# reazon-research/ReazonSpeech

Measured on AMD Instinct MI355X. Metric: RTFx (audio-sec/wall-sec), FastConformer-RNNT 619M batch=256, higher is better.
Workload: dtype bf16

## Files before the change

reazonspeech_amd/csrc/k_frontend.hip:

```cpp
#include "rs_common.h"
#include "k_fft512.h"

namespace {

constexpr int NFFT = FFT512_N;
constexpr int NBIN = FFT512_NBIN;
constexpr int FB_MAXW = 32;
constexpr int WAVES = 4;
constexpr int FRAMES_PER_WAVE = 4;
constexpr int MAX_HOP = 256;
constexpr int SPAN_MAX = (WAVES * FRAMES_PER_WAVE - 1) * MAX_HOP + NFFT;

struct FrontParams {
    const float* audio; const int32_t* lens; float* raw; int32_t* n_frames;
    const float* window;
    const float* twiddle;
    const int32_t* fb_idx;
    const float* fb_w;
    int audio_stride, pad_left, pad_right, t_max, n_mels, win_length, hop;
    float preemph, log_guard;
    int kind;
};

__device__ __forceinline__ float fetch_sample(const float* __restrict__ a, int i, int pad_left, int len) {
    const int j = i - pad_left;
    return (j >= 0 && j < len) ? a[j] : 0.0f;
}

__global__ __launch_bounds__(64 * WAVES) void logmel_kernel(FrontParams p) {
    __shared__ float2 buf[WAVES][FFT512_BUF];
    __shared__ float pw[WAVES][2][NBIN + 3];
    __shared__ float2 tw[NFFT / 2];
    __shared__ float ys[SPAN_MAX];
    __shared__ float win_s[NFFT];
    const int lane = threadIdx.x & 63, wave = threadIdx.x >> 6;
    const int b = blockIdx.y;
    const int len = p.lens[b];
    const int Lp = len + p.pad_left + p.pad_right;
    const int n_valid = p.kind == 2 ? (Lp + p.hop / 2) / p.hop
                                    : Lp / p.hop + (p.kind == 1 ? 1 : 0);
    if (blockIdx.x == 0 && threadIdx.x == 0) p.n_frames[b] = n_valid;
    const float* a = p.audio + (size_t)b * p.audio_stride;
    if ((int)blockIdx.x * WAVES * FRAMES_PER_WAVE >= min(n_valid, p.t_max)) return;
    tw[threadIdx.x] = reinterpret_cast<const float2*>(p.twiddle)[threadIdx.x];
    const int centre_off = (NFFT - p.win_length) / 2;
    const int f0 = blockIdx.x * WAVES * FRAMES_PER_WAVE;
    const int i_base = p.kind == 2 ? f0 * p.hop + p.hop / 2 - p.win_length / 2 : f0 * p.hop - NFFT / 2 + centre_off;
    const int span = (WAVES * FRAMES_PER_WAVE - 1) * p.hop + NFFT;
    for (int idx = threadIdx.x; idx < span; idx += blockDim.x) {
        int i = i_base + idx;
        float y = 0.0f;
        if (p.kind == 1 && Lp > 1) {
            i = i < 0 ? -i : i;
            i = i >= Lp ? 2 * (Lp - 1) - i : i;
            i = i < 0 ? 0 : i;
        }
        if (p.kind == 2 && Lp > 0) {
            for (int bounce = 0; bounce < 8 && (i < 0 || i >= Lp); ++bounce) i = i < 0 ? -i - 1 : 2 * Lp - 1 - i;
            i = i < 0 ? 0 : (i >= Lp ? Lp - 1 : i);
        }
        if (i >= 0 && i < Lp) {
            const float x0 = fetch_sample(a, i, p.pad_left, len);
            if (p.kind == 2) y = x0;
            else y = i >= 1 ? x0 - p.preemph * fetch_sample(a, i - 1, p.pad_left, len) : x0;
        }
        ys[idx] = y;
    }
    for (int idx = threadIdx.x; idx < NFFT; idx += blockDim.x) win_s[idx] = idx < p.win_length ? p.window[idx] : 0.0f;
    __syncthreads();
    const int frame_base = (blockIdx.x * WAVES + wave) * FRAMES_PER_WAVE;
    auto wave_sync = [&]() { fft512_wave_sync(); };
    auto sample = [&](int t, int n) -> float {
        if (t >= n_valid || t >= p.t_max) return 0.0f;
        return ys[(t - f0) * p.hop + n] * win_s[n];
    };
    auto frame_mean = [&](int t) -> float {
        if (t >= n_valid || t >= p.t_max) return 0.0f;
        float sm = 0.0f;
        for (int n = lane; n < p.win_length; n += 64) sm += ys[(t - f0) * p.hop + n];
        return wave_sum(sm) / (float)p.win_length;
    };
    auto sample_kaldi = [&](int t, int n, float mean) -> float {
        if (t >= n_valid || t >= p.t_max || n >= p.win_length) return 0.0f;
        const float* fr = ys + (t - f0) * p.hop;
        const float cur = fr[n] - mean, prev = fr[n > 0 ? n - 1 : 0] - mean;
        return (cur - p.preemph * prev) * win_s[n];
    };

    for (int fi = 0; fi < FRAMES_PER_WAVE; fi += 2) {
        const int t = frame_base + fi;
        if (t >= n_valid || t >= p.t_max) break;
        float2* z = buf[wave];
        float2 v[8];
        if (p.kind == 2) {
            const float m0 = frame_mean(t), m1 = frame_mean(t + 1);
#pragma unroll
            for (int k = 0; k < 8; ++k) v[k] = make_float2(sample_kaldi(t, lane + 64 * k, m0), sample_kaldi(t + 1, lane + 64 * k, m1));
        } else {
#pragma unroll
            for (int k = 0; k < 8; ++k) v[k] = make_float2(sample(t, lane + 64 * k), sample(t + 1, lane + 64 * k));
        }
        fft512_pair(v, z, tw, lane);
        fft512_split_power(z, pw[wave][0], pw[wave][1], lane);
        for (int idx = lane; idx < 2 * p.n_mels; idx += 64) {
            const int f = idx >= p.n_mels, m = idx - f * p.n_mels;
            if (t + f < n_valid && t + f < p.t_max) {
                const int k0 = p.fb_idx[2 * m], cnt = p.fb_idx[2 * m + 1];
                const float* w = p.fb_w + m * FB_MAXW;
                float acc = 0.0f;
                for (int j = 0; j < cnt; ++j) acc = fmaf(w[j], pw[wave][f][k0 + j], acc);
                p.raw[((size_t)b * p.t_max + t + f) * p.n_mels + m] = p.kind >= 1 ? logf(fmaxf(acc, p.log_guard)) : logf(acc + p.log_guard);
            }
        }
        wave_sync();
    }
}

__global__ __launch_bounds__(1024) void feat_normalize_kernel(const float* __restrict__ raw,
                                                              const int32_t* __restrict__ n_frames, int t_max,
                                                              int n_mels, float eps, float* __restrict__ out) {
    __shared__ float4 red[1024];
    __shared__ float4 mean_s[32], rstd_s[32];
    const int b = blockIdx.x;
    const int n = min(n_frames[b], t_max);
    const int Q = n_mels >> 2;
    const int RG = 1000 / Q;
    const int tid = threadIdx.x;
    const int q = tid % Q, rg = tid / Q;
    const bool act = rg < RG;
    const float4* r4 = reinterpret_cast<const float4*>(raw + (size_t)b * t_max * n_mels);
    auto reduce_rows = [&](float4 v) -> float4 {
        red[tid] = act ? v : make_float4(0.f, 0.f, 0.f, 0.f);
        __syncthreads();
        float4 acc = make_float4(0.f, 0.f, 0.f, 0.f);
        if (tid < Q) {
            for (int g = 0; g < RG; ++g) {
                const float4 x = red[g * Q + tid];
                acc.x += x.x; acc.y += x.y; acc.z += x.z; acc.w += x.w;
            }
        }
        return acc;
    };
    float4 s = make_float4(0.f, 0.f, 0.f, 0.f);
    if (act)
#pragma unroll 8
        for (int t = rg; t < n; t += RG) {
            const float4 x = r4[(size_t)t * Q + q];
            s.x += x.x; s.y += x.y; s.z += x.z; s.w += x.w;
        }
    s = reduce_rows(s);
    if (tid < Q) {
        const float inv = 1.0f / (float)n;
        mean_s[tid] = make_float4(s.x * inv, s.y * inv, s.z * inv, s.w * inv);
    }
    __syncthreads();
    const float4 mean = mean_s[q];
    float4 m2 = make_float4(0.f, 0.f, 0.f, 0.f);
    if (act)
#pragma unroll 8
        for (int t = rg; t < n; t += RG) {
            const float4 x = r4[(size_t)t * Q + q];
            const float a = x.x - mean.x, bb = x.y - mean.y, c = x.z - mean.z, d = x.w - mean.w;
            m2.x += a * a; m2.y += bb * bb; m2.z += c * c; m2.w += d * d;
        }
    m2 = reduce_rows(m2);
    if (tid < Q) {
        const float dn = (float)(n - 1);
        rstd_s[tid] = n > 1 ? make_float4(1.0f / (sqrtf(m2.x / dn) + eps), 1.0f / (sqrtf(m2.y / dn) + eps),
                                          1.0f / (sqrtf(m2.z / dn) + eps), 1.0f / (sqrtf(m2.w / dn) + eps))
                            : make_float4(0.f, 0.f, 0.f, 0.f);
    }
    __syncthreads();
    const float4 rstd = rstd_s[q];
    float4* o4 = reinterpret_cast<float4*>(out + (size_t)b * t_max * n_mels);
    if (act)
#pragma unroll 8
        for (int t = rg; t < t_max; t += RG) {
            float4 y = make_float4(0.f, 0.f, 0.f, 0.f);
            if (t < n) {
                const float4 x = r4[(size_t)t * Q + q];
                y = make_float4((x.x - mean.x) * rstd.x, (x.y - mean.y) * rstd.y, (x.z - mean.z) * rstd.z,
                                (x.w - mean.w) * rstd.w);
            }
            o4[(size_t)t * Q + q] = y;
        }
}

__global__ __launch_bounds__(256) void feat_mvn_kernel(const float* __restrict__ raw, const int32_t* __restrict__ n_frames, int t_max,
                                                       int n_mels, const float* __restrict__ mean, const float* __restrict__ istd,
                                                       float* __restrict__ out) {
    const int b = blockIdx.y;
    const int i = blockIdx.x * 256 + threadIdx.x;
    if (i >= t_max * n_mels) return;
    const int t = i / n_mels, m = i - t * n_mels;
    const size_t at = (size_t)b * t_max * n_mels + i;
    out[at] = t < n_frames[b] ? (raw[at] - mean[m]) * istd[m] : 0.0f;
}

}

int rs_launch_frontend(rs_ctx* ctx, const float* audio, const int32_t* lens, int B, int audio_stride,
                       int pad_left, int pad_right, int t_max, float* feats, int32_t* n_frames, float* raw,
                       hipStream_t s) {
    const rs_dims& d = ctx->d;
    if (B <= 0 || t_max <= 0) return RS_OK;
    if (d.n_fft != NFFT) return rs_fail(ctx, RS_EINVAL, "frontend: only n_fft=512 is built");
    if (d.n_mels > 128 || d.n_mels % 4 || d.win_length > NFFT || d.hop_length < 1 || d.hop_length > MAX_HOP)
        return rs_fail(ctx, RS_EINVAL, "frontend: n_mels must be a multiple of 4 up to 128, win <= 512, hop <= %d", MAX_HOP);
    FrontParams p;
    p.audio = audio; p.lens = lens; p.raw = raw; p.n_frames = n_frames;
    p.window = ctx->fe_window; p.twiddle = ctx->fe_twiddle; p.fb_idx = ctx->fe_fb_idx; p.fb_w = ctx->fe_fb_w;
    p.audio_stride = audio_stride; p.pad_left = pad_left; p.pad_right = pad_right; p.t_max = t_max;
    p.n_mels = d.n_mels; p.win_length = d.win_length; p.hop = d.hop_length;
    p.preemph = d.preemph; p.log_guard = d.log_guard;
    p.kind = d.frontend_kind;
    const int fpb = WAVES * FRAMES_PER_WAVE;
    const dim3 grid((t_max + fpb - 1) / fpb, B), block(64 * WAVES);
    if (d.frontend_kind == 2) {
        p.raw = feats;
        RS_HIP(ctx, hipMemsetAsync(feats, 0, (size_t)B * t_max * d.n_mels * 4, s));
    }
    const double bytes = (double)B * ((double)t_max * d.hop_length * 4.0 + (double)t_max * d.n_mels * 4.0 * 3.0);
    rs_prof_scope prof(ctx, RS_PROF_FRONTEND, s, (double)B * t_max * (5.0 * 512 * 9 + 3 * 257 + 2 * 600), bytes);
    hipLaunchKernelGGL(logmel_kernel, grid, block, 0, s, p);
    if (d.frontend_kind == 2) {
    } else if (d.frontend_kind == 1) {
        const rs_conformer& cf = *rs_conformer_of(ctx);
        hipLaunchKernelGGL(feat_mvn_kernel, dim3((t_max * d.n_mels + 255) / 256, B), dim3(256), 0, s, raw, n_frames, t_max, d.n_mels,
                           cf.fe_mvn_mean, cf.fe_mvn_istd, feats);
    } else
        hipLaunchKernelGGL(feat_normalize_kernel, dim3(B), dim3(1024), 0, s, raw, n_frames, t_max, d.n_mels, d.norm_eps,
                           feats);
    prof.end();
    RS_CHECK_LAUNCH(ctx, "frontend");
    return RS_OK;
}
```

reazonspeech_amd/csrc/k_subsample.hip:

```cpp
#include "rs_common.h"

namespace {

__global__ void enc_lens_kernel(const int32_t* __restrict__ n_frames, int B, int stages, int sub_kind, int32_t* __restrict__ out) {
    const int b = blockIdx.x * blockDim.x + threadIdx.x;
    if (b >= B) return;
    int n = n_frames[b];
    for (int s = 0; s < stages; ++s) {
        n = n > 0 ? (sub_kind ? (n >= 3 ? (n - 3) / 2 + 1 : 0) : (n + 2 - 3) / 2 + 1) : 0;
        out[s * B + b] = n;
    }
}

__device__ __forceinline__ void put(uint16_t* p, float v) { *p = f32_to_bf16(v); }
__device__ __forceinline__ void put(float* p, float v) { *p = v; }

template <typename OT>
__global__ __launch_bounds__(256) void sub_conv0_dw1_kernel(
    const float* __restrict__ feats, const int32_t* __restrict__ lens_stage , int B, int t_max,
    int n_mels, int T2, int F1, int F2, int C, const float* __restrict__ w0 ,
    const float* __restrict__ b0, const float* __restrict__ wd , const float* __restrict__ bd,
    OT* __restrict__ out) {
    const int b = blockIdx.y, t2 = blockIdx.x, c = threadIdx.x;
    const int L1 = lens_stage[0 * B + b], L2 = lens_stage[1 * B + b];
    OT* orow = out + (((size_t)b * T2 + t2) * F2) * C + c;
    if (t2 >= L2) {
        for (int f2 = 0; f2 < F2; ++f2) put(orow + (size_t)f2 * C, 0.0f);
        return;
    }
    float k0[9], kd[9];
#pragma unroll
    for (int j = 0; j < 9; ++j) { k0[j] = w0[j * C + c]; kd[j] = wd[j * C + c]; }
    const float bias0 = b0[c], biasd = bd[c];
    const float* fb = feats + (size_t)b * t_max * n_mels;

    const float* rowp[7];
    bool rowok[7];
#pragma unroll
    for (int r = 0; r < 7; ++r) {
        const int tm = 4 * t2 - 3 + r;
        rowok[r] = tm >= 0 && tm < t_max;
        rowp[r] = fb + (size_t)(tm < 0 ? 0 : (tm >= t_max ? t_max - 1 : tm)) * n_mels;
    }
    float kz[3][9];
    bool a_ok[3];
#pragma unroll
    for (int a = 0; a < 3; ++a) {
        const int t1 = 2 * t2 - 1 + a;
        a_ok[a] = t1 >= 0 && t1 < L1;
#pragma unroll
        for (int i = 0; i < 3; ++i)
#pragma unroll
            for (int j = 0; j < 3; ++j) kz[a][i * 3 + j] = rowok[2 * a + i] ? k0[i * 3 + j] : 0.0f;
    }
    float carry[7];
#pragma unroll
    for (int r = 0; r < 7; ++r) carry[r] = 0.0f;
    float left[3];
#pragma unroll
    for (int a = 0; a < 3; ++a) left[a] = 0.0f;
    for (int f2 = 0; f2 < F2; ++f2) {
        float m[7][5];
#pragma unroll
        for (int r = 0; r < 7; ++r) {
            const float4 q = *reinterpret_cast<const float4*>(rowp[r] + 4 * f2);
            m[r][0] = carry[r]; m[r][1] = q.x; m[r][2] = q.y; m[r][3] = q.z; m[r][4] = q.w;
            carry[r] = q.w;
        }
        float mid[3], right[3];
#pragma unroll
        for (int a = 0; a < 3; ++a) {
            float am = 0.0f, ar = 0.0f;
            if (a_ok[a]) {
                am = bias0; ar = bias0;
#pragma unroll
                for (int i = 0; i < 3; ++i)
#pragma unroll
                    for (int j = 0; j < 3; ++j) {
                        am = fmaf(kz[a][i * 3 + j], m[2 * a + i][j], am);
                        ar = fmaf(kz[a][i * 3 + j], m[2 * a + i][2 + j], ar);
                    }
                am = fmaxf(am, 0.0f); ar = fmaxf(ar, 0.0f);
            }
            mid[a] = am; right[a] = ar;
        }
        float acc = biasd;
#pragma unroll
        for (int a = 0; a < 3; ++a) {
            acc = fmaf(kd[a * 3 + 0], left[a], acc);
            acc = fmaf(kd[a * 3 + 1], mid[a], acc);
            acc = fmaf(kd[a * 3 + 2], right[a], acc);
        }
        put(orow + (size_t)f2 * C, acc);
#pragma unroll
        for (int a = 0; a < 3; ++a) left[a] = right[a];
    }
}

__global__ __launch_bounds__(256) void sub_dw_kernel(const uint16_t* __restrict__ in, const float* __restrict__ w ,
                                                     const float* __restrict__ bias, const int32_t* __restrict__ lens_out,
                                                     int Tin, int Fin, int Tout, int Fout, int C,
                                                     uint16_t* __restrict__ out) {
    const int cgs = C >> 3;
    const int cg = threadIdx.x % cgs, fl = threadIdx.x / cgs, fpb = blockDim.x / cgs;
    const int fo = blockIdx.x * fpb + fl, to = blockIdx.y, b = blockIdx.z;
    if (fo >= Fout) return;
    const int c = cg * 8;
    uint16_t* op = out + (((size_t)b * Tout + to) * Fout + fo) * C + c;
    u16x8_t o;
    if (to >= lens_out[b]) {
#pragma unroll
        for (int e = 0; e < 8; ++e) o[e] = 0;
        *reinterpret_cast<u16x8_t*>(op) = o;
        return;
    }
    float acc[8];
    {
        const float4 b0 = reinterpret_cast<const float4*>(bias + c)[0], b1 = reinterpret_cast<const float4*>(bias + c)[1];
        acc[0] = b0.x; acc[1] = b0.y; acc[2] = b0.z; acc[3] = b0.w; acc[4] = b1.x; acc[5] = b1.y; acc[6] = b1.z; acc[7] = b1.w;
    }
#pragma unroll
    for (int i = 0; i < 3; ++i) {
        const int ti = 2 * to - 1 + i;
        if (ti < 0 || ti >= Tin) continue;
#pragma unroll
        for (int j = 0; j < 3; ++j) {
            const int fi = 2 * fo - 1 + j;
            if (fi < 0 || fi >= Fin) continue;
            const u16x8_t x = *reinterpret_cast<const u16x8_t*>(in + (((size_t)b * Tin + ti) * Fin + fi) * C + c);
            const float4 w0 = reinterpret_cast<const float4*>(w + (i * 3 + j) * C + c)[0];
            const float4 w1 = reinterpret_cast<const float4*>(w + (i * 3 + j) * C + c)[1];
            acc[0] = fmaf(w0.x, bf16_to_f32(x[0]), acc[0]); acc[1] = fmaf(w0.y, bf16_to_f32(x[1]), acc[1]);
            acc[2] = fmaf(w0.z, bf16_to_f32(x[2]), acc[2]); acc[3] = fmaf(w0.w, bf16_to_f32(x[3]), acc[3]);
            acc[4] = fmaf(w1.x, bf16_to_f32(x[4]), acc[4]); acc[5] = fmaf(w1.y, bf16_to_f32(x[5]), acc[5]);
            acc[6] = fmaf(w1.z, bf16_to_f32(x[6]), acc[6]); acc[7] = fmaf(w1.w, bf16_to_f32(x[7]), acc[7]);
        }
    }
#pragma unroll
    for (int e = 0; e < 8; ++e) o[e] = f32_to_bf16(acc[e]);
    *reinterpret_cast<u16x8_t*>(op) = o;
}

__global__ __launch_bounds__(256) void sub_dw_f32_kernel(const float* __restrict__ in, const float* __restrict__ w ,
                                                         const float* __restrict__ bias, const int32_t* __restrict__ lens_out,
                                                         int Tin, int Fin, int Tout, int Fout, int C, float* __restrict__ out) {
    const int c = threadIdx.x, fo = blockIdx.x, to = blockIdx.y, b = blockIdx.z;
    float* op = out + (((size_t)b * Tout + to) * Fout + fo) * C + c;
    if (to >= lens_out[b]) { *op = 0.0f; return; }
    float acc = bias[c];
#pragma unroll
    for (int i = 0; i < 3; ++i) {
        const int ti = 2 * to - 1 + i;
        if (ti < 0 || ti >= Tin) continue;
#pragma unroll
        for (int j = 0; j < 3; ++j) {
            const int fi = 2 * fo - 1 + j;
            if (fi < 0 || fi >= Fin) continue;
            acc = fmaf(w[(i * 3 + j) * C + c], in[(((size_t)b * Tin + ti) * Fin + fi) * C + c], acc);
        }
    }
    *op = acc;
}

}

int rs_launch_enc_lens(rs_ctx* ctx, const int32_t* n_frames, int B, int32_t* lens_out, hipStream_t s) {
    hipLaunchKernelGGL(enc_lens_kernel, dim3((B + 127) / 128), dim3(128), 0, s, n_frames, B, ctx->d.sub_stages, ctx->d.sub_kind, lens_out);
    RS_CHECK_LAUNCH(ctx, "enc_lens");
    return RS_OK;
}

int rs_launch_sub_conv0_dw1(rs_ctx* ctx, const float* feats, const int32_t* lens_stage, int B, int t_max, int T2,
                            int F2, uint16_t* out, hipStream_t s) {
    const rs_dims& d = ctx->d;
    const rs_conformer& cf = *rs_conformer_of(ctx);
    const int C = d.sub_channels;
    if (C > 256 || (C % 64)) return rs_fail(ctx, RS_EINVAL, "subsampling: channels %d unsupported (<=256, %%64)", C);
    const int F1 = (d.n_mels + 2 - 3) / 2 + 1;
    if (d.n_mels % 4 || 4 * F2 > d.n_mels || 2 * F2 < F1)
        return rs_fail(ctx, RS_EINVAL, "subsampling: n_mels=%d must be a multiple of 4 with 4*F2 <= n_mels", d.n_mels);
    const size_t lds = 0;
    const double flops = (double)B * T2 * F2 * C * 2.0 * (6 * 9 + 9);
    const double bytes = (double)B * t_max * d.n_mels * 4.0 + (double)B * T2 * F2 * C * 2.0;
    rs_prof_scope prof(ctx, RS_PROF_SUBSAMPLE, s, flops, bytes);
    hipLaunchKernelGGL(sub_conv0_dw1_kernel<uint16_t>, dim3(T2, B), dim3(C), lds, s, feats, lens_stage, B, t_max, d.n_mels, T2,
                       F1, F2, C, cf.sub_conv0_w, cf.sub_conv0_b, cf.sub_dw_w[0], cf.sub_dw_b[0], out);
    prof.end();
    RS_CHECK_LAUNCH(ctx, "sub_conv0_dw1");
    return RS_OK;
}

int rs_launch_sub_dw(rs_ctx* ctx, const uint16_t* in, const float* w, const float* b, const int32_t* lens_out,
                     int stage, int B, int t_in, int f_in, int t_out, int f_out, uint16_t* out, hipStream_t s) {
    (void)stage;
    const int C = ctx->d.sub_channels;
    const int cgs = C / 8;
    const int fpb = 256 / cgs;
    const dim3 grid((f_out + fpb - 1) / fpb, t_out, B), block(cgs * fpb);
    const double bytes = (double)B * C * 2.0 * ((double)t_in * f_in + (double)t_out * f_out);
    rs_prof_scope prof(ctx, RS_PROF_SUBSAMPLE, s, (double)B * t_out * f_out * C * 18.0, bytes);
    hipLaunchKernelGGL(sub_dw_kernel, grid, block, 0, s, in, w, b, lens_out, t_in, f_in, t_out, f_out, C, out);
    prof.end();
    RS_CHECK_LAUNCH(ctx, "sub_dw");
    return RS_OK;
}

int rs_launch_sub_conv0_dw1_f32(rs_ctx* ctx, const float* feats, const int32_t* lens_stage, int B, int t_max, int T2, int F2,
                                float* out, hipStream_t s) {
    const rs_dims& d = ctx->d;
    const rs_conformer& cf = *rs_conformer_of(ctx);
    const int C = d.sub_channels;
    if (C > 256 || (C % 64)) return rs_fail(ctx, RS_EINVAL, "subsampling: channels %d unsupported (<=256, %%64)", C);
    const int F1 = (d.n_mels + 2 - 3) / 2 + 1;
    if (d.n_mels % 4 || 4 * F2 > d.n_mels || 2 * F2 < F1)
        return rs_fail(ctx, RS_EINVAL, "subsampling: n_mels=%d must be a multiple of 4 with 4*F2 <= n_mels", d.n_mels);
    rs_prof_scope prof(ctx, RS_PROF_SUBSAMPLE, s, (double)B * T2 * F2 * C * 2.0 * (6 * 9 + 9),
                       (double)B * t_max * d.n_mels * 4.0 + (double)B * T2 * F2 * C * 4.0);
    hipLaunchKernelGGL(sub_conv0_dw1_kernel<float>, dim3(T2, B), dim3(C), 0, s, feats, lens_stage, B, t_max, d.n_mels, T2, F1, F2, C,
                       cf.sub_conv0_w, cf.sub_conv0_b, cf.sub_dw_w[0], cf.sub_dw_b[0], out);
    prof.end();
    RS_CHECK_LAUNCH(ctx, "sub_conv0_dw1_f32");
    return RS_OK;
}

int rs_launch_sub_dw_f32(rs_ctx* ctx, const float* in, const float* w, const float* b, const int32_t* lens_out, int B, int t_in,
                         int f_in, int t_out, int f_out, float* out, hipStream_t s) {
    const int C = ctx->d.sub_channels;
    rs_prof_scope prof(ctx, RS_PROF_SUBSAMPLE, s, (double)B * t_out * f_out * C * 18.0,
                       (double)B * C * 4.0 * ((double)t_in * f_in + (double)t_out * f_out));
    hipLaunchKernelGGL(sub_dw_f32_kernel, dim3(f_out, t_out, B), dim3(C), 0, s, in, w, b, lens_out, t_in, f_in, t_out, f_out, C, out);
    prof.end();
    RS_CHECK_LAUNCH(ctx, "sub_dw_f32");
    return RS_OK;
}
```

reazonspeech_amd/csrc/rs_knobs.h:

```cpp
#pragma once
#include <stdlib.h>
#include <string.h>

#include <atomic>
#include <mutex>

#include "../../include/rs_asr.h"

#define RS_KNOBS(X)                                                                                                                   \
    X(GEMM_TILE, "RS_GEMM_TILE", INT, 0, "forced GEMM tile height (256 / 192 / 128 / 64); 0 = by shape")                              \
    X(GEMM_GROUP_M, "RS_GEMM_GROUP_M", INT, 0, "row panels per XCD tile group; 0 = by shape")                                         \
    X(GEMM_PAIRS, "RS_GEMM_PAIRS", INT, 2, "2 = two tiles per workgroup, LDS ring carried over; 1 = ring restarted; 0 = one tile")    \
    X(GEMM_BREG, "RS_GEMM_BREG", INT, 0, "1 = 256- / 192-row launches keep the weight operand out of LDS (global -> VGPR)")           \
    X(ATTN_PERSIST, "RS_ATTN_PERSIST", INT, 0, "1 = full attention on resident workgroups that walk the items (n >= 2: on n)")        \
    X(ATTN_STREAM, "RS_ATTN_STREAM", INT, 0, "1 = the streaming attention form (+ 16 x mask: phases left out, for timing)")           \
    X(ATTN64, "RS_ATTN64", INT, 4, "head_dim 64: key blocks per chunk; 0 = the one-workgroup-per-CU geometry")                        \
    X(ATTN64_NW, "RS_ATTN64_NW", INT, 4, "head_dim 64: waves per workgroup (the second number of $RS_ATTN64)")                        \
    X(ATTN_F32_OLD, "RS_ATTN_F32_OLD", PRESENT, 0, "float32 attention: the first form (one wave per key sum)")                        \
    X(ATTN_F32_KEYS, "RS_ATTN_F32_KEYS", PRESENT, 0, "float32 attention: the second form (keys over lanes, no MFMA)")                 \
    X(GLU_GENERIC, "RS_GLU_GENERIC", INT, 0, "GLU + depthwise conv: 1 = the any-kernel-size path, 2 = the f32-tile kernel on the gated layout") \
    X(SUB_IM2COL, "RS_SUB_IM2COL", PRESENT, 0, "ESPnet subsampling: gather the 3 x 3 patches into a matrix first (sizes the workspace too)") \
    X(FUSE_GLU, "RS_FUSE_GLU", INT, 1, "context default: 0 = GLU in the depthwise kernel, not the pw1 GEMM epilogue")                 \
    X(DEFER_OUT_NORM, "RS_DEFER_OUT_NORM", INT, 1, "context default: 0 = every output norm stores its f32 rows")                      \
    X(DECODE_SCREEN, "RS_DECODE_SCREEN", INT, 1, "context default: 0 = exact evaluation of every joint column")                       \
    X(DECODE_NARROW, "RS_DECODE_NARROW", INT, 1, "context default: 0 = the wide-tile LSTM / projection kernels")                      \
    X(DECODE_NO_XCD, "RS_DECODE_NO_XCD", PRESENT, 0, "greedy decode: joint grids not padded to a multiple of 8 column tiles")         \
    X(DECODE_NO_LOOKAHEAD, "RS_DECODE_NO_LOOKAHEAD", PRESENT, 0, "greedy decode: one frame per utterance and step at every batch size") \
    X(VERIFY_WIDE, "RS_VERIFY_WIDE", INT, 0, "screened joint: 1 = a workgroup per row for V <= 3072 too")                             \
    X(DECODE_TRACE, "RS_DECODE_TRACE", PRESENT, 0, "greedy decode: print the step count of every call to stderr")                     \
    X(BEAM_SPEC, "RS_BEAM_SPEC", INT, 3, "beam search: evaluations asked for per iteration (1 .. 8; sizes the workspace too)")         \
    X(BEAM_TRACE, "RS_BEAM_TRACE", PRESENT, 0, "beam search: phase timing of the step kernel")                                        \
    X(BEAM_RECORD_LDS, "RS_BEAM_RECORD_LDS", PRESENT, 0, "beam search: the any-vocabulary record kernel on a small vocabulary")       \
    X(AVSR_POSCONV_OLD, "RS_AVSR_POSCONV_OLD", PRESENT, 0, "AV-HuBERT positional convolution: the VALU form")                         \
    X(K2_CONV1_OLD, "RS_K2_CONV1_OLD", PRESENT, 0, "Zipformer conv1: the VALU form (the one other channel counts run)")               \
    X(K2_ATTW_SWEEPS, "RS_K2_ATTW_SWEEPS", INT, 1, "Zipformer attention weights: 3 = the three-sweep kernel")                         \
    X(K2_CONV2_FUSED, "RS_K2_CONV2_FUSED", INT, 1, "default of option k2_conv2_fused: 0 = patch matrix + GEMM launch")                \
    X(K2_CNX_FUSED, "RS_K2_CNX_FUSED", INT, 1, "default of option k2_cnx_fused: 0 = the ConvNeXt pointwise pair as two GEMM launches")

enum rs_knob_id {
#define RS_KNOB_ENUM(id, env, kind, def, what) RS_KNOB_##id,
    RS_KNOBS(RS_KNOB_ENUM)
#undef RS_KNOB_ENUM
    RS_KNOB_COUNT
};
enum rs_knob_kind { RS_KNOB_PRESENT, RS_KNOB_INT };
struct rs_knob_row { const char* env; rs_knob_kind kind; int def; };
static const rs_knob_row rs_knob_rows[RS_KNOB_COUNT] = {
#define RS_KNOB_ROW(id, env, kind, def, what) {env, RS_KNOB_##kind, def},
    RS_KNOBS(RS_KNOB_ROW)
#undef RS_KNOB_ROW
};

struct rs_knob_table {
    std::atomic<int> value[RS_KNOB_COUNT];
    std::atomic<bool> given[RS_KNOB_COUNT];
    std::once_flag once;
};
inline rs_knob_table rs_knob_state;

inline void rs_knobs_read_env() {
    std::call_once(rs_knob_state.once, [] {
        rs_knob_table& t = rs_knob_state;
        for (int i = 0; i < RS_KNOB_COUNT; ++i) { t.value[i] = rs_knob_rows[i].def; t.given[i] = false; }
        for (int i = 0; i < RS_KNOB_COUNT; ++i) {
            const char* e = i == RS_KNOB_ATTN64_NW ? nullptr : getenv(rs_knob_rows[i].env);
            if (!e) continue;
            t.given[i] = true;
            t.value[i] = rs_knob_rows[i].kind == RS_KNOB_PRESENT ? 1 : atoi(e);
            if (i == RS_KNOB_ATTN64) {
                t.given[RS_KNOB_ATTN64_NW] = true;
                if (const char* c = strchr(e, ',')) t.value[RS_KNOB_ATTN64_NW] = atoi(c + 1);
            }
        }
    });
}

inline int rs_knob(rs_knob_id id) { rs_knobs_read_env(); return rs_knob_state.value[id].load(std::memory_order_relaxed); }
inline bool rs_knob_given(rs_knob_id id) { rs_knobs_read_env(); return rs_knob_state.given[id].load(std::memory_order_relaxed); }
inline void rs_knob_set(rs_knob_id id, int v) { rs_knobs_read_env(); rs_knob_state.value[id].store(v, std::memory_order_relaxed); }

inline int rs_knob_find(const char* env_name) {
    for (int i = 0; env_name && i < RS_KNOB_COUNT; ++i)
        if (!strcmp(env_name, rs_knob_rows[i].env)) return i;
    return -1;
}
inline int rs_knob_set_named(const char* env_name, int v) {
    const int i = rs_knob_find(env_name);
    if (i < 0) return RS_EINVAL;
    rs_knob_set((rs_knob_id)i, v);
    return RS_OK;
}
inline int rs_knob_get_named(const char* env_name, int* v) {
    const int i = rs_knob_find(env_name);
    if (i < 0 || !v) return RS_EINVAL;
    *v = rs_knob((rs_knob_id)i);
    return RS_OK;
}
```

Before: 45670.

## Add lean log-mel and row-run subsampling kernels reusing conv rows across time

```diff
diff --git a/reazonspeech_amd/csrc/k_frontend.hip b/reazonspeech_amd/csrc/k_frontend.hip
--- a/reazonspeech_amd/csrc/k_frontend.hip
+++ b/reazonspeech_amd/csrc/k_frontend.hip
@@ -27,12 +27,17 @@
     return (j >= 0 && j < len) ? a[j] : 0.0f;
 }
 
+constexpr int MEL_PASSES = 4;
+template <bool LEAN>
 __global__ __launch_bounds__(64 * WAVES) void logmel_kernel(FrontParams p) {
     __shared__ float2 buf[WAVES][FFT512_BUF];
     __shared__ float pw[WAVES][2][NBIN + 3];
     __shared__ float2 tw[NFFT / 2];
-    __shared__ float ys[SPAN_MAX];
-    __shared__ float win_s[NFFT];
+    __shared__ float ys_first[LEAN ? 1 : SPAN_MAX];
+    __shared__ float win_first[LEAN ? 1 : NFFT];
+    extern __shared__ float lean_lds[];
+    float* const ys = LEAN ? lean_lds : ys_first;
+    float* const win_s = win_first;
     const int lane = threadIdx.x & 63, wave = threadIdx.x >> 6;
     const int b = blockIdx.y;
     const int len = p.lens[b];
@@ -47,9 +52,30 @@
     const int f0 = blockIdx.x * WAVES * FRAMES_PER_WAVE;
     const int i_base = p.kind == 2 ? f0 * p.hop + p.hop / 2 - p.win_length / 2 : f0 * p.hop - NFFT / 2 + centre_off;
     const int span = (WAVES * FRAMES_PER_WAVE - 1) * p.hop + NFFT;
-    for (int idx = threadIdx.x; idx < span; idx += blockDim.x) {
+    const int fb_pitch = p.n_mels + 1;
+    float* const fbw_s = lean_lds + span;
+    float wreg[8];
+    int it_m[MEL_PASSES], it_k0[MEL_PASSES], it_cnt[MEL_PASSES];
+    int cnt_max = 0;
+    if constexpr (LEAN) {
+#pragma unroll 5
+        for (int e = threadIdx.x; e < p.n_mels * FB_MAXW; e += blockDim.x)
+            fbw_s[(e % FB_MAXW) * fb_pitch + e / FB_MAXW] = p.fb_w[e];
+#pragma unroll
+        for (int k = 0; k < 8; ++k) wreg[k] = lane + 64 * k < p.win_length ? p.window[lane + 64 * k] : 0.0f;
+#pragma unroll
+        for (int q = 0; q < MEL_PASSES; ++q) {
+            const int idx = lane + 64 * q;
+            const bool on = idx < 2 * p.n_mels;
+            const int m = on ? idx - (idx >= p.n_mels ? p.n_mels : 0) : 0;
+            it_m[q] = m;
+            it_k0[q] = on ? p.fb_idx[2 * m] : 0;
+            it_cnt[q] = on ? min(p.fb_idx[2 * m + 1], FB_MAXW) : 0;
+            cnt_max = max(cnt_max, it_cnt[q]);
+        }
+    }
+    auto padded_index = [&](int idx) -> int {
         int i = i_base + idx;
-        float y = 0.0f;
         if (p.kind == 1 && Lp > 1) {
             i = i < 0 ? -i : i;
             i = i >= Lp ? 2 * (Lp - 1) - i : i;
@@ -59,6 +85,38 @@
             for (int bounce = 0; bounce < 8 && (i < 0 || i >= Lp); ++bounce) i = i < 0 ? -i - 1 : 2 * Lp - 1 - i;
             i = i < 0 ? 0 : (i >= Lp ? Lp - 1 : i);
         }
+        return i;
+    };
+    if constexpr (LEAN) {
+        constexpr int STAGE_CHUNK = 12;
+        for (int base = 0; base < span; base += STAGE_CHUNK * 64 * WAVES) {
+            float r0[STAGE_CHUNK], r1[STAGE_CHUNK];
+#pragma unroll
+            for (int k = 0; k < STAGE_CHUNK; ++k) {
+                const int j = padded_index(base + k * 64 * WAVES + (int)threadIdx.x) - p.pad_left;
+                r0[k] = 0.0f; r1[k] = 0.0f;
+                if (len > 0) {
+                    r0[k] = a[min(max(j, 0), len - 1)];
+                    if (p.kind != 2) r1[k] = a[min(max(j - 1, 0), len - 1)];
+                }
+            }
+#pragma unroll
+            for (int k = 0; k < STAGE_CHUNK; ++k) {
+                const int idx = base + k * 64 * WAVES + (int)threadIdx.x;
+                const int i = padded_index(idx), j = i - p.pad_left;
+                float y = 0.0f;
+                if (i >= 0 && i < Lp) {
+                    const float x0 = (j >= 0 && j < len) ? r0[k] : 0.0f;
+                    if (p.kind == 2) y = x0;
+                    else y = i >= 1 ? x0 - p.preemph * ((j - 1 >= 0 && j - 1 < len) ? r1[k] : 0.0f) : x0;
+                }
+                if (idx < span) ys[idx] = y;
+            }
+        }
+    } else
+    for (int idx = threadIdx.x; idx < span; idx += blockDim.x) {
+        int i = padded_index(idx);
+        float y = 0.0f;
         if (i >= 0 && i < Lp) {
             const float x0 = fetch_sample(a, i, p.pad_left, len);
             if (p.kind == 2) y = x0;
@@ -66,7 +124,12 @@
         }
         ys[idx] = y;
     }
-    for (int idx = threadIdx.x; idx < NFFT; idx += blockDim.x) win_s[idx] = idx < p.win_length ? p.window[idx] : 0.0f;
+    if constexpr (LEAN) {
+#pragma unroll
+        for (int off = 32; off > 0; off >>= 1) cnt_max = max(cnt_max, __shfl_xor(cnt_max, off, 64));
+        cnt_max = __builtin_amdgcn_readfirstlane(cnt_max);
+    } else
+        for (int idx = threadIdx.x; idx < NFFT; idx += blockDim.x) win_s[idx] = idx < p.win_length ? p.window[idx] : 0.0f;
     __syncthreads();
     const int frame_base = (blockIdx.x * WAVES + wave) * FRAMES_PER_WAVE;
     auto wave_sync = [&]() { fft512_wave_sync(); };
@@ -74,6 +137,10 @@
         if (t >= n_valid || t >= p.t_max) return 0.0f;
         return ys[(t - f0) * p.hop + n] * win_s[n];
     };
+    auto sample_lean = [&](int t, int k) -> float {
+        if (t >= n_valid || t >= p.t_max) return 0.0f;
+        return ys[(t - f0) * p.hop + lane + 64 * k] * wreg[k];
+    };
     auto frame_mean = [&](int t) -> float {
         if (t >= n_valid || t >= p.t_max) return 0.0f;
         float sm = 0.0f;
@@ -86,13 +153,29 @@
         const float cur = fr[n] - mean, prev = fr[n > 0 ? n - 1 : 0] - mean;
         return (cur - p.preemph * prev) * win_s[n];
     };
+    auto sample_kaldi_lean = [&](int t, int k, float mean) -> float {
+        const int n = lane + 64 * k;
+        if (t >= n_valid || t >= p.t_max || n >= p.win_length) return 0.0f;
+        const float* fr = ys + (t - f0) * p.hop;
+        const float cur = fr[n] - mean, prev = fr[n > 0 ? n - 1 : 0] - mean;
+        return (cur - p.preemph * prev) * wreg[k];
+    };
 
     for (int fi = 0; fi < FRAMES_PER_WAVE; fi += 2) {
         const int t = frame_base + fi;
         if (t >= n_valid || t >= p.t_max) break;
         float2* z = buf[wave];
         float2 v[8];
-        if (p.kind == 2) {
+        if constexpr (LEAN) {
+            if (p.kind == 2) {
+                const float m0 = frame_mean(t), m1 = frame_mean(t + 1);
+#pragma unroll
+                for (int k = 0; k < 8; ++k) v[k] = make_float2(sample_kaldi_lean(t, k, m0), sample_kaldi_lean(t + 1, k, m1));
+            } else {
+#pragma unroll
+                for (int k = 0; k < 8; ++k) v[k] = make_float2(sample_lean(t, k), sample_lean(t + 1, k));
+            }
+        } else if (p.kind == 2) {
             const float m0 = frame_mean(t), m1 = frame_mean(t + 1);
 #pragma unroll
             for (int k = 0; k < 8; ++k) v[k] = make_float2(sample_kaldi(t, lane + 64 * k, m0), sample_kaldi(t + 1, lane + 64 * k, m1));
@@ -102,6 +185,24 @@
         }
         fft512_pair(v, z, tw, lane);
         fft512_split_power(z, pw[wave][0], pw[wave][1], lane);
+        if constexpr (LEAN) {
+#pragma unroll
+            for (int q = 0; q < MEL_PASSES; ++q) {
+                if (64 * q >= 2 * p.n_mels) break;
+                const int idx = lane + 64 * q;
+                const int f = idx >= p.n_mels, m = it_m[q], k0 = it_k0[q], cnt = it_cnt[q];
+                const float* pwr = pw[wave][f];
+                const float* wcol = fbw_s + m;
+                float acc = 0.0f;
+#pragma unroll 6
+                for (int j = 0; j < cnt_max; ++j) {
+                    const float next = fmaf(wcol[j * fb_pitch], pwr[min(k0 + j, NBIN - 1)], acc);
+                    acc = j < cnt ? next : acc;
+                }
+                if (idx < 2 * p.n_mels && t + f < n_valid && t + f < p.t_max)
+                    p.raw[((size_t)b * p.t_max + t + f) * p.n_mels + m] = p.kind >= 1 ? logf(fmaxf(acc, p.log_guard)) : logf(acc + p.log_guard);
+            }
+        } else
         for (int idx = lane; idx < 2 * p.n_mels; idx += 64) {
             const int f = idx >= p.n_mels, m = idx - f * p.n_mels;
             if (t + f < n_valid && t + f < p.t_max) {
@@ -222,7 +323,12 @@
     }
     const double bytes = (double)B * ((double)t_max * d.hop_length * 4.0 + (double)t_max * d.n_mels * 4.0 * 3.0);
     rs_prof_scope prof(ctx, RS_PROF_FRONTEND, s, (double)B * t_max * (5.0 * 512 * 9 + 3 * 257 + 2 * 600), bytes);
-    hipLaunchKernelGGL(logmel_kernel, grid, block, 0, s, p);
+    if (rs_knob(RS_KNOB_LOGMEL_OLD))
+        hipLaunchKernelGGL(logmel_kernel<false>, grid, block, 0, s, p);
+    else {
+        const size_t lds = ((size_t)(fpb - 1) * d.hop_length + NFFT + (size_t)FB_MAXW * (d.n_mels + 1)) * sizeof(float);
+        hipLaunchKernelGGL(logmel_kernel<true>, grid, block, lds, s, p);
+    }
     if (d.frontend_kind == 2) {
     } else if (d.frontend_kind == 1) {
         const rs_conformer& cf = *rs_conformer_of(ctx);
diff --git a/reazonspeech_amd/csrc/k_subsample.hip b/reazonspeech_amd/csrc/k_subsample.hip
--- a/reazonspeech_amd/csrc/k_subsample.hip
+++ b/reazonspeech_amd/csrc/k_subsample.hip
@@ -97,6 +97,157 @@
     }
 }
 
+constexpr int SUB_RUN = 12;
+
+typedef float f32x2_t __attribute__((ext_vector_type(2)));
+__device__ __forceinline__ f32x2_t vfma(f32x2_t a, f32x2_t b, f32x2_t c) { return __builtin_elementwise_fma(a, b, c); }
+__device__ __forceinline__ f32x2_t vfma(f32x2_t a, float b, f32x2_t c) { const f32x2_t bb = {b, b}; return __builtin_elementwise_fma(a, bb, c); }
+__device__ __forceinline__ f32x2_t vrelu(f32x2_t a) { const f32x2_t r = {fmaxf(a.x, 0.0f), fmaxf(a.y, 0.0f)}; return r; }
+__device__ __forceinline__ void vload(const float* p, f32x2_t& v) { v = *reinterpret_cast<const f32x2_t*>(p); }
+__device__ __forceinline__ void put(uint16_t* p, f32x2_t v) {
+    const unsigned u = (unsigned)f32_to_bf16(v.x) | ((unsigned)f32_to_bf16(v.y) << 16);
+    *reinterpret_cast<unsigned*>(p) = u;
+}
+__device__ __forceinline__ void put(float* p, f32x2_t v) { *reinterpret_cast<f32x2_t*>(p) = v; }
+
+template <typename OT, int F2C>
+__global__ __launch_bounds__(256) void sub_conv0_dw1_run_kernel(
+    const float* __restrict__ feats, const int32_t* __restrict__ lens_stage , int B, int t_max,
+    int n_mels, int T2, int C, const float* __restrict__ w0 , const float* __restrict__ b0,
+    const float* __restrict__ wd , const float* __restrict__ bd, OT* __restrict__ out) {
+    using V = f32x2_t;
+    const int b = blockIdx.y, t2_first = blockIdx.x * SUB_RUN, c = threadIdx.x * 2;
+    const int L1 = lens_stage[0 * B + b], L2 = lens_stage[1 * B + b];
+    const int t2_end = min(t2_first + SUB_RUN, T2);
+    const int t2_live = min(t2_end, L2);
+    OT* obase = out + ((size_t)b * T2 * F2C) * C + c;
+    const V zero = {};
+    if (t2_first < t2_live) {
+        V k0[9], kd[9];
+#pragma unroll
+        for (int j = 0; j < 9; ++j) { vload(w0 + j * C + c, k0[j]); vload(wd + j * C + c, kd[j]); }
+        V bias0, biasd;
+        vload(b0 + c, bias0); vload(bd + c, biasd);
+        const float* fb = feats + (size_t)b * t_max * n_mels;
+        float touched = 0.0f;
+        auto touch = [&](int tm_first) -> float {
+            const int at = tm_first * n_mels + (int)threadIdx.x * 16;
+            return (int)threadIdx.x * 16 < 5 * n_mels ? fb[min(max(at, 0), t_max * n_mels - 1)] : 0.0f;
+        };
+        const float touched_first = touch(4 * t2_first - 1);
+        V cm[F2C], cr[F2C];
+        {
+            const int t1 = 2 * t2_first - 1;
+#pragma unroll
+            for (int f2 = 0; f2 < F2C; ++f2) { cm[f2] = zero; cr[f2] = zero; }
+            if (t1 >= 0 && t1 < L1) {
+                const float* rowp[3];
+                V kz[9];
+#pragma unroll
+                for (int i = 0; i < 3; ++i) {
+                    const int tm = 2 * t1 - 1 + i;
+                    const bool ok = tm >= 0 && tm < t_max;
+                    rowp[i] = fb + (size_t)(tm < 0 ? 0 : (tm >= t_max ? t_max - 1 : tm)) * n_mels;
+#pragma unroll
+                    for (int j = 0; j < 3; ++j) kz[i * 3 + j] = ok ? k0[i * 3 + j] : zero;
+                }
+                float carry[3] = {0.0f, 0.0f, 0.0f};
+#pragma unroll
+                for (int f2 = 0; f2 < F2C; ++f2) {
+                    float m[3][5];
+#pragma unroll
+                    for (int i = 0; i < 3; ++i) {
+                        const float4 q = *reinterpret_cast<const float4*>(rowp[i] + 4 * f2);
+                        m[i][0] = carry[i]; m[i][1] = q.x; m[i][2] = q.y; m[i][3] = q.z; m[i][4] = q.w;
+                        carry[i] = q.w;
+                    }
+                    V am = bias0, ar = bias0;
+#pragma unroll
+                    for (int i = 0; i < 3; ++i)
+#pragma unroll
+                        for (int j = 0; j < 3; ++j) {
+                            am = vfma(kz[i * 3 + j], m[i][j], am);
+                            ar = vfma(kz[i * 3 + j], m[i][2 + j], ar);
+                        }
+                    cm[f2] = vrelu(am); cr[f2] = vrelu(ar);
+                }
+            }
+        }
+        for (int t2 = t2_first; t2 < t2_live; ++t2) {
+            const float touched_next = touch(4 * t2 + 3);
+            const float* rowp[5];
+            bool rowok[5];
+#pragma unroll
+            for (int r = 0; r < 5; ++r) {
+                const int tm = 4 * t2 - 1 + r;
+                rowok[r] = tm >= 0 && tm < t_max;
+                rowp[r] = fb + (size_t)(tm < 0 ? 0 : (tm >= t_max ? t_max - 1 : tm)) * n_mels;
+            }
+            V kz[2][9];
+            bool a_ok[2];
+#pragma unroll
+            for (int a = 0; a < 2; ++a) {
+                const int t1 = 2 * t2 + a;
+                a_ok[a] = t1 >= 0 && t1 < L1;
+#pragma unroll
+                for (int i = 0; i < 3; ++i)
+#pragma unroll
+                    for (int j = 0; j < 3; ++j) kz[a][i * 3 + j] = rowok[2 * a + i] ? k0[i * 3 + j] : zero;
+            }
+            float carry[5];
+#pragma unroll
+            for (int r = 0; r < 5; ++r) carry[r] = 0.0f;
+            V left[3] = {zero, zero, zero};
+            OT* orow = obase + ((size_t)t2 * F2C) * C;
+#pragma unroll
+            for (int f2 = 0; f2 < F2C; ++f2) {
+                float m[5][5];
+#pragma unroll
+                for (int r = 0; r < 5; ++r) {
+                    const float4 q = *reinterpret_cast<const float4*>(rowp[r] + 4 * f2);
+                    m[r][0] = carry[r]; m[r][1] = q.x; m[r][2] = q.y; m[r][3] = q.z; m[r][4] = q.w;
+                    carry[r] = q.w;
+                }
+                V mid[3], right[3];
+                mid[0] = cm[f2]; right[0] = cr[f2];
+#pragma unroll
+                for (int a = 0; a < 2; ++a) {
+                    V am = zero, ar = zero;
+                    if (a_ok[a]) {
+                        am = bias0; ar = bias0;
+#pragma unroll
+                        for (int i = 0; i < 3; ++i)
+#pragma unroll
+                            for (int j = 0; j < 3; ++j) {
+                                am = vfma(kz[a][i * 3 + j], m[2 * a + i][j], am);
+                                ar = vfma(kz[a][i * 3 + j], m[2 * a + i][2 + j], ar);
+                            }
+                        am = vrelu(am); ar = vrelu(ar);
+                    }
+                    mid[a + 1] = am; right[a + 1] = ar;
+                }
+                V acc = biasd;
+#pragma unroll
+                for (int a = 0; a < 3; ++a) {
+                    acc = vfma(kd[a * 3 + 0], left[a], acc);
+                    acc = vfma(kd[a * 3 + 1], mid[a], acc);
+                    acc = vfma(kd[a * 3 + 2], right[a], acc);
+                }
+                put(orow + (size_t)f2 * C, acc);
+#pragma unroll
+                for (int a = 0; a < 3; ++a) left[a] = right[a];
+                cm[f2] = mid[2]; cr[f2] = right[2];
+            }
+            touched += touched_next;
+        }
+        if (touched + touched_first == 1.0e-30f && t_max < 0) put(obase, zero);
+    }
+    for (int t2 = max(t2_first, t2_live); t2 < t2_end; ++t2) {
+        OT* orow = obase + ((size_t)t2 * F2C) * C;
+        for (int f2 = 0; f2 < F2C; ++f2) put(orow + (size_t)f2 * C, zero);
+    }
+}
+
 __global__ __launch_bounds__(256) void sub_dw_kernel(const uint16_t* __restrict__ in, const float* __restrict__ w ,
                                                      const float* __restrict__ bias, const int32_t* __restrict__ lens_out,
                                                      int Tin, int Fin, int Tout, int Fout, int C,
@@ -141,6 +292,93 @@
     *reinterpret_cast<u16x8_t*>(op) = o;
 }
 
+constexpr int DW_RUN = 6;
+
+__device__ __forceinline__ void dw_taps(float (&acc)[8], const float (&wt)[9][8], int i, const u16x8_t (&x)[3], const bool (&jok)[3]) {
+#pragma unroll
+    for (int j = 0; j < 3; ++j) {
+        if (!jok[j]) continue;
+#pragma unroll
+        for (int e = 0; e < 8; ++e) acc[e] = fmaf(wt[i * 3 + j][e], bf16_to_f32(x[j][e]), acc[e]);
+    }
+}
+
+__global__ __launch_bounds__(512) void sub_dw_run_kernel(const uint16_t* __restrict__ in, const float* __restrict__ w ,
+                                                         const float* __restrict__ bias, const int32_t* __restrict__ lens_out,
+                                                         int Tin, int Fin, int Tout, int Fout, int C,
+                                                         uint16_t* __restrict__ out) {
+    const int cgs = C >> 3;
+    const int cg = threadIdx.x % cgs, fo = threadIdx.x / cgs;
+    const int b = blockIdx.y, to_first = blockIdx.x * DW_RUN;
+    const int c = cg * 8;
+    const int to_end = min(to_first + DW_RUN, Tout);
+    const int to_live = min(to_end, lens_out[b]);
+    uint16_t* obase = out + (((size_t)b * Tout) * Fout + fo) * C + c;
+    if (to_first < to_live) {
+        float wt[9][8], bs[8];
+#pragma unroll
+        for (int k = 0; k < 9; ++k) {
+            const float4 w0 = reinterpret_cast<const float4*>(w + k * C + c)[0], w1 = reinterpret_cast<const float4*>(w + k * C + c)[1];
+            wt[k][0] = w0.x; wt[k][1] = w0.y; wt[k][2] = w0.z; wt[k][3] = w0.w; wt[k][4] = w1.x; wt[k][5] = w1.y; wt[k][6] = w1.z; wt[k][7] = w1.w;
+        }
+        {
+            const float4 b0 = reinterpret_cast<const float4*>(bias + c)[0], b1 = reinterpret_cast<const float4*>(bias + c)[1];
+            bs[0] = b0.x; bs[1] = b0.y; bs[2] = b0.z; bs[3] = b0.w; bs[4] = b1.x; bs[5] = b1.y; bs[6] = b1.z; bs[7] = b1.w;
+        }
+        bool jok[3];
+#pragma unroll
+        for (int j = 0; j < 3; ++j) { const int fi = 2 * fo - 1 + j; jok[j] = fi >= 0 && fi < Fin; }
+        const uint16_t* ibase = in + ((size_t)b * Tin * Fin) * C + c;
+        auto load_row = [&](int ti, u16x8_t (&x)[3]) {
+#pragma unroll
+            for (int j = 0; j < 3; ++j) {
+                if (jok[j]) x[j] = *reinterpret_cast<const u16x8_t*>(ibase + ((size_t)ti * Fin + (2 * fo - 1 + j)) * C);
+                else
+#pragma unroll
+                    for (int e = 0; e < 8; ++e) x[j][e] = 0;
+            }
+        };
+        u16x8_t top[3], mid[3], bot[3];
+#pragma unroll
+        for (int j = 0; j < 3; ++j)
+#pragma unroll
+            for (int e = 0; e < 8; ++e) { top[j][e] = 0; mid[j][e] = 0; bot[j][e] = 0; }
+        bool top_ok = to_first > 0 && 2 * to_first - 1 < Tin;
+        if (top_ok) load_row(2 * to_first - 1, top);
+        u16x8_t mid_next[3], bot_next[3];
+#pragma unroll
+        for (int j = 0; j < 3; ++j) { mid_next[j] = mid[j]; bot_next[j] = bot[j]; }
+        if (2 * to_first < Tin) load_row(2 * to_first, mid_next);
+        if (2 * to_first + 1 < Tin) load_row(2 * to_first + 1, bot_next);
+        for (int to = to_first; to < to_live; ++to) {
+            const bool mid_ok = 2 * to < Tin, bot_ok = 2 * to + 1 < Tin;
+#pragma unroll
+            for (int j = 0; j < 3; ++j) { mid[j] = mid_next[j]; bot[j] = bot_next[j]; }
+            if (to + 1 < to_live) {
+                if (2 * to + 2 < Tin) load_row(2 * to + 2, mid_next);
+                if (2 * to + 3 < Tin) load_row(2 * to + 3, bot_next);
+            }
+            float acc[8];
+#pragma unroll
+            for (int e = 0; e < 8; ++e) acc[e] = bs[e];
+            if (top_ok) dw_taps(acc, wt, 0, top, jok);
+            if (mid_ok) dw_taps(acc, wt, 1, mid, jok);
+            if (bot_ok) dw_taps(acc, wt, 2, bot, jok);
+            u16x8_t o;
+#pragma unroll
+            for (int e = 0; e < 8; ++e) o[e] = f32_to_bf16(acc[e]);
+            *reinterpret_cast<u16x8_t*>(obase + ((size_t)to * Fout) * C) = o;
+#pragma unroll
+            for (int j = 0; j < 3; ++j) top[j] = bot[j];
+            top_ok = bot_ok;
+        }
+    }
+    u16x8_t z;
+#pragma unroll
+    for (int e = 0; e < 8; ++e) z[e] = 0;
+    for (int to = max(to_first, to_live); to < to_end; ++to) *reinterpret_cast<u16x8_t*>(obase + ((size_t)to * Fout) * C) = z;
+}
+
 __global__ __launch_bounds__(256) void sub_dw_f32_kernel(const float* __restrict__ in, const float* __restrict__ w ,
                                                          const float* __restrict__ bias, const int32_t* __restrict__ lens_out,
                                                          int Tin, int Fin, int Tout, int Fout, int C, float* __restrict__ out) {
@@ -169,6 +407,9 @@
     RS_CHECK_LAUNCH(ctx, "enc_lens");
     return RS_OK;
 }
+
+constexpr int SUB_F2 = 20;
+static bool conv0_run_form(int F2) { return F2 == SUB_F2 && !rs_knob(RS_KNOB_SUB_CONV0_OLD); }
 
 int rs_launch_sub_conv0_dw1(rs_ctx* ctx, const float* feats, const int32_t* lens_stage, int B, int t_max, int T2,
                             int F2, uint16_t* out, hipStream_t s) {
@@ -183,7 +424,11 @@
     const double flops = (double)B * T2 * F2 * C * 2.0 * (6 * 9 + 9);
     const double bytes = (double)B * t_max * d.n_mels * 4.0 + (double)B * T2 * F2 * C * 2.0;
     rs_prof_scope prof(ctx, RS_PROF_SUBSAMPLE, s, flops, bytes);
-    hipLaunchKernelGGL(sub_conv0_dw1_kernel<uint16_t>, dim3(T2, B), dim3(C), lds, s, feats, lens_stage, B, t_max, d.n_mels, T2,
+    if (conv0_run_form(F2))
+        hipLaunchKernelGGL((sub_conv0_dw1_run_kernel<uint16_t, SUB_F2>), dim3((T2 + SUB_RUN - 1) / SUB_RUN, B), dim3(C / 2), lds, s, feats,
+                           lens_stage, B, t_max, d.n_mels, T2, C, cf.sub_conv0_w, cf.sub_conv0_b, cf.sub_dw_w[0], cf.sub_dw_b[0], out);
+    else
+        hipLaunchKernelGGL(sub_conv0_dw1_kernel<uint16_t>, dim3(T2, B), dim3(C), lds, s, feats, lens_stage, B, t_max, d.n_mels, T2,
                        F1, F2, C, cf.sub_conv0_w, cf.sub_conv0_b, cf.sub_dw_w[0], cf.sub_dw_b[0], out);
     prof.end();
     RS_CHECK_LAUNCH(ctx, "sub_conv0_dw1");
@@ -199,7 +444,11 @@
     const dim3 grid((f_out + fpb - 1) / fpb, t_out, B), block(cgs * fpb);
     const double bytes = (double)B * C * 2.0 * ((double)t_in * f_in + (double)t_out * f_out);
     rs_prof_scope prof(ctx, RS_PROF_SUBSAMPLE, s, (double)B * t_out * f_out * C * 18.0, bytes);
-    hipLaunchKernelGGL(sub_dw_kernel, grid, block, 0, s, in, w, b, lens_out, t_in, f_in, t_out, f_out, C, out);
+    if (!rs_knob(RS_KNOB_SUB_DW_OLD) && cgs * f_out <= 512)
+        hipLaunchKernelGGL(sub_dw_run_kernel, dim3((t_out + DW_RUN - 1) / DW_RUN, B), dim3(cgs * f_out), 0, s, in, w, b, lens_out, t_in,
+                           f_in, t_out, f_out, C, out);
+    else
+        hipLaunchKernelGGL(sub_dw_kernel, grid, block, 0, s, in, w, b, lens_out, t_in, f_in, t_out, f_out, C, out);
     prof.end();
     RS_CHECK_LAUNCH(ctx, "sub_dw");
     return RS_OK;
@@ -216,7 +465,11 @@
         return rs_fail(ctx, RS_EINVAL, "subsampling: n_mels=%d must be a multiple of 4 with 4*F2 <= n_mels", d.n_mels);
     rs_prof_scope prof(ctx, RS_PROF_SUBSAMPLE, s, (double)B * T2 * F2 * C * 2.0 * (6 * 9 + 9),
                        (double)B * t_max * d.n_mels * 4.0 + (double)B * T2 * F2 * C * 4.0);
-    hipLaunchKernelGGL(sub_conv0_dw1_kernel<float>, dim3(T2, B), dim3(C), 0, s, feats, lens_stage, B, t_max, d.n_mels, T2, F1, F2, C,
+    if (conv0_run_form(F2))
+        hipLaunchKernelGGL((sub_conv0_dw1_run_kernel<float, SUB_F2>), dim3((T2 + SUB_RUN - 1) / SUB_RUN, B), dim3(C / 2), 0, s, feats,
+                           lens_stage, B, t_max, d.n_mels, T2, C, cf.sub_conv0_w, cf.sub_conv0_b, cf.sub_dw_w[0], cf.sub_dw_b[0], out);
+    else
+        hipLaunchKernelGGL(sub_conv0_dw1_kernel<float>, dim3(T2, B), dim3(C), 0, s, feats, lens_stage, B, t_max, d.n_mels, T2, F1, F2, C,
                        cf.sub_conv0_w, cf.sub_conv0_b, cf.sub_dw_w[0], cf.sub_dw_b[0], out);
     prof.end();
     RS_CHECK_LAUNCH(ctx, "sub_conv0_dw1_f32");
diff --git a/reazonspeech_amd/csrc/rs_knobs.h b/reazonspeech_amd/csrc/rs_knobs.h
--- a/reazonspeech_amd/csrc/rs_knobs.h
+++ b/reazonspeech_amd/csrc/rs_knobs.h
@@ -31,6 +31,9 @@
     X(BEAM_SPEC, "RS_BEAM_SPEC", INT, 3, "beam search: evaluations asked for per iteration (1 .. 8; sizes the workspace too)")         \
     X(BEAM_TRACE, "RS_BEAM_TRACE", PRESENT, 0, "beam search: phase timing of the step kernel")                                        \
     X(BEAM_RECORD_LDS, "RS_BEAM_RECORD_LDS", PRESENT, 0, "beam search: the any-vocabulary record kernel on a small vocabulary")       \
+    X(LOGMEL_OLD, "RS_LOGMEL_OLD", PRESENT, 0, "log-mel: the first form (16 frames per workgroup, filterbank read from global memory)") \
+    X(SUB_CONV0_OLD, "RS_SUB_CONV0_OLD", PRESENT, 0, "conv0 + dw1: the first form (a workgroup per output row, every odd conv0 row twice)") \
+    X(SUB_DW_OLD, "RS_SUB_DW_OLD", PRESENT, 0, "bf16 depthwise stage: the first form (a thread per output bin, every input row read by two rows)") \
     X(AVSR_POSCONV_OLD, "RS_AVSR_POSCONV_OLD", PRESENT, 0, "AV-HuBERT positional convolution: the VALU form")                         \
     X(K2_CONV1_OLD, "RS_K2_CONV1_OLD", PRESENT, 0, "Zipformer conv1: the VALU form (the one other channel counts run)")               \
     X(K2_ATTW_SWEEPS, "RS_K2_ATTW_SWEEPS", INT, 1, "Zipformer attention weights: 3 = the three-sweep kernel")                         \
```

New measurement: 46280, median of 6. +1.3%, better.
